# ZhongLingXiao/nano-kazen

Hardware: AMD Instinct MI355X
Metric: Msamples/s (w*h*spp/s) at 1920x1080, 1 M-tri scene (higher is better)
Workload: dtype f32

## Files before the change

### nano-kazen_amd/csrc/kz_render.hip

```cpp
#include <hip/hip_runtime.h>

#include "kz_devfn.h"
#include "kz_wavefront.h"
#include "kz_integrators.h"
#include "kz_aov.h"
#include "kz_state.h"
#include "../../include/kazen_mi355x_variance.h"
#include <algorithm>
#include <cmath>
#include <cstring>
#include <mutex>
#include <string>

template <bool STATS, int EXT>
__global__ __launch_bounds__(KZ_BLOCK) void kz_path_megakernel(KzParams P, KzDevTables T, const uint32_t *__restrict__ pixList,
                                                               uint32_t nItems, uint32_t S, uint32_t sampleBegin, const uint32_t *__restrict__ itemSample,
                                                               float *__restrict__ outJx, float *__restrict__ outJy, float *__restrict__ outR,
                                                               float *__restrict__ outG, float *__restrict__ outB,
                                                               unsigned long long *__restrict__ stats) {
    __shared__ uint32_t s_stack[KZ_STACK_DEPTH * KZ_BLOCK];
    const uint32_t item = blockIdx.x * KZ_BLOCK + threadIdx.x;
    Counters cn = {0, 0, 0, 0, 0, 0};
    if (item < nItems) {
        const uint32_t pl = item / S, so = item - pl * S;
// ... 24 lines not shown
}

static int stageMark(PassCtx &c, hipStream_t stream, int kind) {
    if (c.stageUsed == c.stageEv.size()) { Event e; if (const int rc = e.ensure()) return rc; c.stageEv.push_back(std::move(e)); c.stageKind.push_back(0); }
    c.stageKind[c.stageUsed] = kind;
    HIP_TRY(hipEventRecord(c.stageEv[c.stageUsed++], stream));
    return KZ_OK;
}

static constexpr size_t KZ_STATE_BYTES_PER_ITEM = 8 * sizeof(float4) + sizeof(uint4) + 3 * sizeof(uint32_t);
static constexpr size_t KZ_SAMPLE_BYTES_PER_ITEM = 5 * sizeof(float);

static void ctxPoint(PassCtx &c, const KzArena &A, size_t off) {
    KzWf W{};
    W.rayA.p = A.array<float4>(0) + off; W.rayB.p = A.array<float4>(1) + off; W.hit.p = A.array<float4>(2) + off; W.thr.p = A.array<float4>(3) + off;
    W.misc.p = A.array<float4>(4) + off; W.shA.p = A.array<float4>(5) + off; W.shB.p = A.array<float4>(6) + off; W.shL.p = A.array<float4>(7) + off;
    W.smp = A.array<uint4>(8) + off;
    for (int q = 0; q < 3; ++q) W.queue[q] = A.array<uint32_t>(9 + q) + off;
    W.counts = c.counts;
    c.wf = W;
    for (int k = 0; k < 5; ++k) c.plane[k] = A.array<float>(12 + k) + off;
}

static int ctxEnsure(PassCtx &c, size_t want, size_t minItems, double graceMs, hipStream_t stream, size_t *usable) {
    if (!c.counts) { if (const int rc = c.counts.alloc(KzCounts::kWords)) return rc; }
    KzArena &A = *c.arena;
    if (A.wouldReallocate(want)) HIP_TRY(hipDeviceSynchronize());
#ifdef KZ_EXPERIMENTS
    if (g_failAlloc > 0) { A.failCountdown.store(g_failAlloc); g_failAlloc = 0; }
#endif
    size_t got = 0;
    const int rc = A.request(want, minItems, graceMs, &got);
#ifdef KZ_EXPERIMENTS
    { std::lock_guard<std::mutex> g(A.m); if (!A.busy) g_failAlloc = A.failCountdown.exchange(0); }
#endif
    if (rc) return rc;
    ctxPoint(c, A, 0);
    *usable = std::min(got, want);
    return KZ_OK;
}

static decltype(&kz_wf_trace<0, false>) traceFn(int mode, bool stats) {
    static const decltype(&kz_wf_trace<0, false>) tab[5][2] = {{kz_wf_trace<0, false>, kz_wf_trace<0, true>}, {kz_wf_trace<1, false>, kz_wf_trace<1, true>},
                                        {kz_wf_trace<2, false>, kz_wf_trace<2, true>}, {nullptr, nullptr}, {kz_wf_trace<4, false>, kz_wf_trace<4, true>}};
#ifdef KZ_EXPERIMENTS
    if (mode == 4 && !g_kzShadowOrder.load(std::memory_order_relaxed)) return stats ? kz_wf_trace<5, true> : kz_wf_trace<5, false>;
#endif
    return tab[mode][stats ? 1 : 0];
}
static decltype(&kz_wf_trace_list<false, false>) listFn(bool stats, bool fix) {
    static const decltype(&kz_wf_trace_list<false, false>) tab[2][2] = {{kz_wf_trace_list<false, false>, kz_wf_trace_list<false, true>}, {kz_wf_trace_list<true, false>, kz_wf_trace_list<true, true>}};
    return tab[stats ? 1 : 0][fix ? 1 : 0];
}
static decltype(&kz_wf_trace_packet<false, false>) packetFn(bool stats, bool fix) {
    static const decltype(&kz_wf_trace_packet<false, false>) tab[2][2] = {{kz_wf_trace_packet<false, false>, kz_wf_trace_packet<false, true>}, {kz_wf_trace_packet<true, false>, kz_wf_trace_packet<true, true>}};
    return tab[stats ? 1 : 0][fix ? 1 : 0];
}
static int extSel(int bsdfExt, int all) { return bsdfExt == 0 ? 0 : (bsdfExt == KZ_X_MODELS ? KZ_X_MODELS : all); }
static int extCol(int ext) { return ext == 0 ? 0 : (ext == KZ_X_MODELS ? 1 : 2); }
typedef decltype(&kz_wf_shade<false, 0>) KzShadeFn;
static KzShadeFn shadeFn(bool stats, int ext) {
    static const KzShadeFn tab[2][3] = {{kz_wf_shade<false, 0>, kz_wf_shade<false, KZ_X_MODELS>, kz_wf_shade<false, KZ_X_ALL>}, {kz_wf_shade<true, 0>, kz_wf_shade<true, KZ_X_MODELS>, kz_wf_shade<true, KZ_X_ALL>}};
    return tab[stats ? 1 : 0][extCol(ext)];
}
typedef decltype(&kz_wf_mats<0>) KzMatsFn;
static KzMatsFn matsFn(int ext) {
    static const KzMatsFn tab[3] = {kz_wf_mats<0>, kz_wf_mats<KZ_X_MODELS>, kz_wf_mats<KZ_X_MATS>};
    return tab[extCol(ext)];
}
typedef decltype(&kz_path_megakernel<false, 0>) KzMegaFn;
static KzMegaFn megaFn(bool stats, int ext) {
    static const KzMegaFn tab[2][2] = {{kz_path_megakernel<false, 0>, kz_path_megakernel<false, KZ_X_ALL>}, {kz_path_megakernel<true, 0>, kz_path_megakernel<true, KZ_X_ALL>}};
    return tab[stats ? 1 : 0][ext ? 1 : 0];
}
typedef decltype(&kz_integrator_megakernel<KZ_INTEGRATOR_NORMALS, 0>) KzIntegratorMegaFn;
static KzIntegratorMegaFn integratorMegaFn(int integrator, int ext) {
    static const KzIntegratorMegaFn tab[3][2] = {{kz_integrator_megakernel<KZ_INTEGRATOR_NORMALS, 0>, kz_integrator_megakernel<KZ_INTEGRATOR_NORMALS, KZ_X_MATS>},
                                                 {kz_integrator_megakernel<KZ_INTEGRATOR_AO, 0>, kz_integrator_megakernel<KZ_INTEGRATOR_AO, KZ_X_MATS>},
                                                 {kz_integrator_megakernel<KZ_INTEGRATOR_PATH_MATS, 0>, kz_integrator_megakernel<KZ_INTEGRATOR_PATH_MATS, KZ_X_MATS>}};
    return tab[integrator == KZ_INTEGRATOR_NORMALS ? 0 : (integrator == KZ_INTEGRATOR_AO ? 1 : 2)][ext ? 1 : 0];
}

static int ensureBeamBuffers(KzScene *scene, KzDeviceState *ds, hipStream_t stream) {
    const KzParams &P = scene->prm;
    const size_t framePix = (size_t)P.width * P.height;
    int rc;
    if ((rc = ds->evBeam.ensure(hipEventDisableTiming))) return rc;
    if (!ds->beamEntries || !ds->beamCount) {
        if (!ds->beamEntries && (rc = ds->beamEntries.alloc(framePix * KZ_BEAM_CAP))) return rc;
        if (!ds->beamCount && (rc = ds->beamCount.alloc(framePix))) return rc;
        HIP_TRY(hipMemsetAsync(ds->beamCount, 0xFF, framePix * sizeof(uint2), stream));
        ds->beamDone.clear(); ds->beamDoneGen = ds->tileGen;
    }
    return KZ_OK;
}
static int ensureBeams(KzScene *scene, KzDeviceState *ds, hipStream_t stream, uint32_t p0, uint32_t n) {
    const KzParams &P = scene->prm;
    { const int rc_ = ensureBeamBuffers(scene, ds, stream); if (rc_) return rc_; }
    if (ds->beamDoneGen != ds->tileGen) { ds->beamDone.clear(); ds->beamDoneGen = ds->tileGen; }
    for (const auto &r : ds->beamDone) if (r.first <= p0 && p0 + n <= r.first + r.second) return KZ_OK;
    const int LS = std::max(1, std::min(P.stackBound4, KZ_BEAM_STACK));
    const dim3 gBeam((n + KZ_BLOCK - 1) / KZ_BLOCK);
    const size_t beamLds = (size_t)2 * LS * KZ_BLOCK * sizeof(uint32_t);
    hipLaunchKernelGGL(kz_wf_beam, gBeam, dim3(KZ_BLOCK), beamLds, stream, P, ds->T, (const uint32_t *)(ds->pixList + p0), n, LS, ds->beamEntries, ds->beamCount);
    if (ds->statsOn) hipLaunchKernelGGL(kz_wf_beam_count, gBeam, dim3(KZ_BLOCK), 0, stream, (const uint2 *)ds->beamCount, (const uint32_t *)(ds->pixList + p0), P.width, n, ds->stats + 24);
    HIP_TRY(hipGetLastError());
// ... 9 lines not shown
static bool packetFits(const KzParams &P) { return P.stackBound4 <= 128; }
struct TraceShape {
    int ldsStack;
    size_t traceLds;
    uint32_t ovfStride;
    size_t ovfRows, ovfPart;
};
static TraceShape traceShape(const KzParams &P, unsigned gridBlocks, int ldsStackAsked) {
    TraceShape s;
    const int stackBound = std::max(P.stackBound4, 2);
    s.ldsStack = std::max(2, std::min(ldsStackAsked, stackBound));
    s.traceLds = (size_t)(s.ldsStack + 1) * KZ_BLOCK * sizeof(uint32_t);
    s.ovfStride = (uint32_t)((size_t)gridBlocks * KZ_BLOCK);
    s.ovfRows = (size_t)std::max(1, stackBound - s.ldsStack);
    s.ovfPart = (size_t)s.ovfStride * s.ovfRows;
    return s;
}
static void launchTrace(int mode, bool stats, dim3 grid, size_t traceLds, hipStream_t on, const KzParams &P, const KzDevTables &T, const KzWf &W, const uint32_t *q, const uint32_t *cptr,
                        uint32_t cimm, uint32_t *head, KzTune t, uint32_t *qb, uint32_t *cb) {
    if (t.batch <= 0) t.batch = 128;
    if (t.refill <= 0) t.refill = (mode == 2 || mode == 4) ? 32 : 40;
    hipLaunchKernelGGL(traceFn(mode, stats), grid, dim3(KZ_BLOCK), traceLds, on, P, T, W, q, cptr, cimm, head, t, qb, cb);
}
template <class Trace>
static void shadowLaunches(const KzParams &P, Trace &&trace, const uint32_t *q, const uint32_t *cptr, uint32_t cimm, uint32_t *head, uint32_t *litQ, uint32_t *litCount, uint32_t *litHead) {
    if (P.shadowFast) {
        trace(4, q, cptr, cimm, head, litQ, litCount);
        if (P.anyInvisibleLight) trace(2, (const uint32_t *)litQ, (const uint32_t *)litCount, 0u, litHead, (uint32_t *)nullptr, (uint32_t *)nullptr);
    } else trace(2, q, cptr, cimm, head, (uint32_t *)nullptr, (uint32_t *)nullptr);
}

static int ensureOverflow(KzScene *scene, KzDeviceState *ds, PassCtx &c, const KzTune &tune, hipStream_t stream) {
    const size_t needOvf = traceShape(scene->prm, travGridBlocks(ds, tune), tune.ldsStack).ovfPart * 3;
    if (needOvf <= c.ovf.cap()) return KZ_OK;
    HIP_TRY(hipStreamSynchronize(stream));
    return c.ovf.regrow(needOvf);
}

struct WfLaunch {
    KzDeviceState *ds; PassCtx &c; hipStream_t stream;
    KzParams P; KzDevTables Tsh; KzWf W; KzTune tune;
    const uint32_t *pixList; uint32_t items, Sp, sBegin; bool st;
    dim3 blk, gItems, gTrav, gShade, gPacket;
    size_t traceLds, ovfPart;
    int mark(int kind) { return stageMark(c, stream, kind); }
    void trace(int mode, const uint32_t *q, const uint32_t *cptr, uint32_t cimm, uint32_t *head, uint32_t *qb, uint32_t *cb, hipStream_t on = nullptr) const {
        KzTune t = tune;
        const bool side = on != nullptr;
        if (side) t.ovf = tune.ovf + 2 * ovfPart; else on = stream;
        launchTrace(mode, st, gTrav, traceLds, on, P, ds->T, W, q, cptr, cimm, head, t, qb, cb);
    }
};

static int wfCamera(WfLaunch &L, bool beams) {
    const KzParams &P = L.P; const KzWf &W = L.W; KzDeviceState *ds = L.ds; hipStream_t stream = L.stream;
    uint32_t *cam = W.counts + KzCounts::kCamera, *fixCount = cam + KzCounts::kPaths;
    const bool packet = L.tune.packet != 1 && packetFits(P), fix = P.anyInvisibleLight != 0;
    if (packet && beams) {
        uint32_t *fbQ = W.queue[0], *fbCount = W.counts + KzCounts::kFallback, *fbHead = fbCount + 1;
        hipLaunchKernelGGL(listFn(L.st, fix), L.gItems, L.blk, 0, stream, P, ds->T, W, L.pixList, L.items, L.Sp, (const uint2 *)ds->beamEntries, (const uint2 *)ds->beamCount,
                           fbQ, fbCount, W.queue[2], fixCount);
        hipLaunchKernelGGL(packetFn(L.st, fix), L.gPacket, L.blk, 0, stream, P, ds->T, W, (const uint32_t *)fbQ, (const uint32_t *)fbCount, 0u, fbHead, KZ_PACKET_BATCH, W.queue[2], fixCount);
    } else if (packet) {
        hipLaunchKernelGGL(packetFn(L.st, fix), L.gPacket, L.blk, 0, stream, P, ds->T, W, (const uint32_t *)nullptr, (const uint32_t *)nullptr, L.items, cam + KzCounts::kBounceHead, KZ_PACKET_BATCH, W.queue[2], fixCount);
    } else {
        L.trace(0, nullptr, nullptr, L.items, cam + KzCounts::kBounceHead, nullptr, nullptr);
        if (fix) hipLaunchKernelGGL(kz_wf_primary_fix, L.gShade, L.blk, 0, stream, P, ds->T, W, L.items, W.queue[2], fixCount);
    }
    if (fix) L.trace(1, W.queue[2], fixCount, 0u, cam + KzCounts::kShadowHead, nullptr, nullptr);
    return L.mark(5);
}

#define KZ_VARIANCE_DEFAULT_ONE_PASS 1
static int filmStages(KzScene *scene, KzDeviceState *ds, hipStream_t pst, const uint32_t *pixList, uint32_t nPix, uint32_t Sp, const float *const plane[5], hipEvent_t waitFilm, int lanes) {
    const int mode = scene->varianceMode;
    if (!mode) return kzFilmStage(scene, ds, ds->picture(), false, pst, pixList, nPix, Sp, plane, waitFilm, lanes);
    const bool onePass = (mode == KZ_VARIANCE_ONE_PASS || (mode == KZ_VARIANCE_ON && KZ_VARIANCE_DEFAULT_ONE_PASS)) && kzFilmMomentOnePassOk(scene->prm);
    if (!onePass) if (const int rc = kzFilmStage(scene, ds, ds->picture(), false, pst, pixList, nPix, Sp, plane, waitFilm, lanes)) return rc;
    return kzFilmStageMoment(scene, ds, ds->picture(), ds->moment(), onePass, pst, pixList, nPix, Sp, plane, waitFilm);
}
static int filmLanes(const KzTune &tune) { return tune.filmGather == 3 ? 1 : 0; }
typedef decltype(&kz_wf_aov<0>) KzAovFn;
static KzAovFn aovFn(int ext) {
    static const KzAovFn tab[3] = {kz_wf_aov<0>, kz_wf_aov<KZ_X_MODELS>, kz_wf_aov<KZ_X_ALL>};
    return tab[extCol(ext)];
}
static int wfAov(KzScene *scene, WfLaunch &L, hipEvent_t waitAov, hipEvent_t recordAov) {
    const KzWf &W = L.W; hipStream_t stream = L.stream;
    static_assert(sizeof(float4) >= 3 * sizeof(float), "a shadow array holds three float planes per item");
    const KzAovPlanes A = {{(float *)W.shA.p, (float *)W.shB.p, (float *)W.shL.p}, (size_t)L.items};
    const dim3 grid(std::min(L.gItems.x, (unsigned)(L.ds->numCU * 8)));
    hipLaunchKernelGGL(aovFn(extSel(L.P.bsdfExt, KZ_X_ALL)), grid, L.blk, 0, stream, L.ds->T, W, L.items, scene->aovMask, A);
    HIP_TRY(hipGetLastError());
    if (waitAov) HIP_TRY(hipStreamWaitEvent(stream, waitAov, 0));
    for (int f = 0; f < 3; ++f) {
        if (!(scene->aovMask & (1u << f))) continue;
        KzFilm &film = L.ds->aov(f);
        if (!film.sums) return kz_fail(KZ_ERR_STATE, "the tap sums of AOV %u are not there", 1u << f);
        const float *const plane[5] = {W.outJx, W.outJy, A.p[f], A.p[f] + A.stride, A.p[f] + 2 * A.stride};
        if (const int rc = kzFilmStage(scene, L.ds, film, true, stream, L.pixList, L.items / L.Sp, L.Sp, plane, nullptr, filmLanes(L.tune))) return rc;
    }
    if (recordAov) HIP_TRY(hipEventRecord(recordAov, stream));
    return L.mark(4);
}

static int wfMats(WfLaunch &L) {
    int rc;
    const KzParams &P = L.P; const KzWf &W = L.W; hipStream_t stream = L.stream;
    const KzMatsFn mats = matsFn(extSel(P.bsdfExt, KZ_X_MATS));
    const uint32_t *cur = nullptr, *curCount = nullptr;
    for (int iter = 0; iter < P.maxDepth; ++iter) {
        uint32_t *nextQ = W.queue[iter & 1], *nextCount = W.counts + KzCounts::quad(iter);
        hipLaunchKernelGGL(mats, L.gShade, L.blk, 0, stream, P, L.ds->T, W, L.pixList, L.Sp, L.sBegin, iter, cur, curCount, cur ? 0u : L.items, nextQ, nextCount);
        if ((rc = L.mark(2))) return rc;
// ... 21 lines not shown
        uint32_t *nextQ = W.queue[iter & 1], *nextCount = W.counts + KzCounts::quad(iter), *shQ = W.queue[2], *shCount = nextCount + KzCounts::kShadows;
        hipLaunchKernelGGL(shade, L.gShade, L.blk, 0, stream, P, L.Tsh, W, L.pixList, L.Sp, L.sBegin, iter, cur, curCount, L.items, nextQ, nextCount, shQ, shCount);
        const bool needExtend = iter < P.maxDepth - 1 || P.bgPresent;
        if ((rc = L.mark(2))) return rc;
        hipStream_t shOn = nullptr;
        if (beside && needExtend) { HIP_TRY(hipEventRecord(c.evFork, stream)); HIP_TRY(hipStreamWaitEvent(c.side, c.evFork, 0)); shOn = c.side; }
        if (P.nLights > 0) {
            uint32_t *litQ = W.queue[(iter & 1) ^ 1], *litCount = W.counts + KzCounts::lit(iter), *litHead = litCount + 1;
            shadowLaunches(P, [&](int mode, const uint32_t *q, const uint32_t *cptr, uint32_t cimm, uint32_t *head, uint32_t *qb, uint32_t *cb) { L.trace(mode, q, cptr, cimm, head, qb, cb, shOn); },
                           shQ, shCount, 0u, nextCount + KzCounts::kShadowHead, litQ, litCount, litHead);
        }
        if (shOn) HIP_TRY(hipEventRecord(c.evJoin, c.side));
        if ((rc = L.mark(3))) return rc;
        if (needExtend) {
            L.trace(0, nextQ, nextCount, 0u, nextCount + KzCounts::kBounceHead, nullptr, nullptr);
            if (shOn) HIP_TRY(hipStreamWaitEvent(stream, c.evJoin, 0));
            if ((rc = L.mark(1))) return rc;
        }
        cur = nextQ; curCount = nextCount;
    }
    if (P.bgPresent) hipLaunchKernelGGL(kz_wf_final, L.gShade, L.blk, 0, stream, P, L.ds->T, W, cur, curCount);
    return KZ_OK;
}

static int wfPass(KzScene *scene, KzDeviceState *ds, PassCtx &c, hipStream_t stream, const uint32_t *pixList, uint32_t sBegin, uint32_t Sp, uint32_t items, KzTune tune, bool beams, bool beside,
                  hipEvent_t waitAov = nullptr, hipEvent_t recordAov = nullptr) {
    int rc;
    WfLaunch L{ds, c, stream};
    const bool mis = scene->prm.integrator == KZ_INTEGRATOR_PATH_MIS;
    KzParams &P = L.P = scene->prm;
    if (!mis) { P.anyInvisibleLight = 0; P.nIlTris = 0; P.shadowFast = 1; }
    L.Tsh = ds->T;
    if (ds->statsOn) L.Tsh.nEmTris = KZ_EM_OFF;
#ifdef KZ_EXPERIMENTS
    { const int mode = g_kzRrAhead.load(std::memory_order_relaxed);
      if (mode == 0) L.Tsh.nEmTris = KZ_EM_OFF; else if (mode == 2) L.Tsh.nEmTris = ds->T.nEmTris; }
#endif
    KzWf &W = L.W = c.wf;
    W.outJx = c.plane[0]; W.outJy = c.plane[1]; W.outR = c.plane[2]; W.outG = c.plane[3]; W.outB = c.plane[4]; W.stats = ds->stats;
    L.pixList = pixList; L.items = items; L.Sp = Sp; L.sBegin = sBegin; L.st = ds->statsOn;
    const int shadeBlocks = tune.shadeBlocksPerCU > 0 ? tune.shadeBlocksPerCU : !mis ? 8 : (P.bsdfExt ? 6 : KZ_SHADE_WAVES);
    L.blk = dim3(KZ_BLOCK); L.gItems = dim3((items + KZ_BLOCK - 1) / KZ_BLOCK);
    L.gTrav = dim3(travGridBlocks(ds, tune)); L.gShade = dim3((unsigned)(ds->numCU * shadeBlocks));
    L.gPacket = dim3(packetGridBlocks(ds));
    const TraceShape shape = traceShape(P, L.gTrav.x, tune.ldsStack);
    tune.ldsStack = shape.ldsStack;
    L.traceLds = shape.traceLds;
    if ((rc = ensureOverflow(scene, ds, c, tune, stream))) return rc;
    tune.ovf = c.ovf; tune.ovfStride = shape.ovfStride;
    L.tune = tune; L.ovfPart = shape.ovfPart;
    c.stageUsed = 0;
    HIP_TRY(hipMemsetAsync(W.counts, 0, KzCounts::bytes(), stream));
    if ((rc = L.mark(-1))) return rc;
    hipLaunchKernelGGL(kz_wf_generate, L.gItems, L.blk, 0, stream, P, ds->T, W, pixList, items, Sp, sBegin);
    if ((rc = L.mark(0))) return rc;
    if (mis && P.maxDepth <= 0 && !scene->aovMask) return KZ_OK;
    if ((rc = wfCamera(L, beams))) return rc;
    if (scene->aovMask && (rc = wfAov(scene, L, waitAov, recordAov))) return rc;
    if (mis && P.maxDepth <= 0) return KZ_OK;
    if (P.integrator == KZ_INTEGRATOR_NORMALS) {
        hipLaunchKernelGGL(kz_wf_normals, L.gShade, L.blk, 0, stream, P, ds->T, W, items);
        rc = L.mark(2);
    } else if (P.integrator == KZ_INTEGRATOR_AO) {
        uint32_t *quad = W.counts + KzCounts::quad(0), *shQ = W.queue[2], *shCount = quad + KzCounts::kShadows;
        hipLaunchKernelGGL(kz_wf_ao, L.gShade, L.blk, 0, stream, P, ds->T, W, pixList, Sp, sBegin, items, shQ, shCount);
        if ((rc = L.mark(2))) return rc;
        L.trace(4, shQ, shCount, 0u, quad + KzCounts::kShadowHead, nullptr, nullptr);
        rc = L.mark(3);
    } else rc = mis ? wfMis(L, beside) : wfMats(L);
    if (rc) return rc;
    if (L.st) hipLaunchKernelGGL(kz_wf_count, L.gItems, L.blk, 0, stream, W, items);
    HIP_TRY(hipGetLastError());
    return KZ_OK;
}

static int planIn(KzDeviceState *ds, const KzRenderOpts *opts, int pipeline, uint32_t s0, uint32_t s1, KzPlanIn &in) {
    in.pipeline = pipeline; in.nPix = ds->nPix; in.s0 = s0; in.s1 = s1;
    in.passItems = opts->passItems; in.passesInFlight = opts->passesInFlight; in.sppPerPass = opts->tune.sppPerPass;
    in.perItem = (pipeline == 2 ? KZ_STATE_BYTES_PER_ITEM : 0) + KZ_SAMPLE_BYTES_PER_ITEM;
    in.limit = opts->maxStateBytes;
    if (!in.limit) {
        size_t freeB = 0, totalB = 0;
        const size_t held = ds->ctxBytes() + kzCtxPoolBytes(ds->device);
        if (hipMemGetInfo(&freeB, &totalB) == hipSuccess && totalB > 0) in.limit = std::min(totalB / 4 * 3, freeB + held - std::min(freeB + held, KzArena::kRuntimeReserve + ((size_t)256 << 20)));
        else in.limit = (size_t)32 << 30;
        if (in.limit == 0) return kz_fail(KZ_ERR_OOM, "the device has %.2f GB free and this replica holds no pass context: nothing is left for path state beyond the %.2f GB a context leaves to the HIP runtime's own allocations",
                                          freeB / 1e9, (KzArena::kRuntimeReserve + ((size_t)256 << 20)) / 1e9);
    }
    const KzTileDealer *dealer = opts->dealer;
    in.dealer = dealer != nullptr;
    if (dealer) { in.takers = dealer->takers; in.dealerBatchTiles = dealer->batchTiles; in.nTiles = (uint32_t)ds->curTiles.size(); in.tilePixOffset = ds->tilePixOffset.data(); }
    in.heldBefore = ds->ctx[0] ? std::max(ds->ctx[0]->wanted, ds->ctx[0]->items()) : kzCtxPoolMaxItems(ds->device);
    return KZ_OK;
}

static int makeRoom(KzDeviceState *ds, int nCtx, size_t need, size_t perItem, size_t limit) {
    const size_t perCtx = need * perItem;
    size_t keep = 0;
    for (int i = 0; i < nCtx; ++i) { PassCtx &c = ds->ctxAt(i); if (c.arena) c.arena->lowerTarget(need); keep += std::max(c.bytes(), perCtx); }
    for (int i = KZ_MAX_PASSES_IN_FLIGHT - 1; i >= nCtx; --i) {
        if (!ds->ctx[i] || !ds->ctx[i]->bytes()) continue;
        if (keep + ds->ctx[i]->bytes() > limit) { HIP_TRY(hipDeviceSynchronize()); ds->ctx[i]->release(); } else keep += ds->ctx[i]->bytes();
    }
    if (keep + kzCtxPoolBytes(ds->device) > limit) (void)kzCtxPoolTrim(ds->device, limit > keep ? limit - keep : 0);
    if (keep > limit)
        for (int i = 0; i < nCtx; ++i) if (ds->ctx[i] && ds->ctx[i]->bytes() > perCtx) {
            HIP_TRY(hipDeviceSynchronize());
// ... 433 lines not shown
```

### nano-kazen_amd/csrc/kz_wavefront.h

```cpp
#pragma once
#include "kz_state.h"
#include "kz_devfn.h"

#ifndef KZ_WF_QCAP
#define KZ_WF_QCAP 960
#endif
#define KZ_WF_ROUNDS (KZ_WF_QCAP / KZ_BLOCK)

struct WfAppender {
    uint32_t *s_buf; uint32_t *s_n; uint32_t *s_gb; uint32_t *gQueue; uint32_t *gCount;
    __device__ __forceinline__ void push(bool pred, uint32_t val) {
        const unsigned long long m = __ballot(pred);
        const int lane = threadIdx.x & 63;
        uint32_t base = 0;
        if (lane == 0 && m) base = atomicAdd(s_n, (uint32_t)__popcll(m));
        base = __shfl(base, 0, 64);
        if (pred) s_buf[base + __popcll(m & ((1ull << lane) - 1ull))] = val;
    }
    __device__ __forceinline__ void maybeFlush(bool force) {
        __syncthreads();
        const uint32_t n = *s_n;
        if (force ? (n > 0) : (n > KZ_WF_QCAP - KZ_BLOCK)) {
            if (threadIdx.x == 0) *s_gb = atomicAdd(gCount, n);
            __syncthreads();
            const uint32_t gb = *s_gb;
            for (uint32_t i = threadIdx.x; i < n; i += KZ_BLOCK) gQueue[gb + i] = s_buf[i];
            __syncthreads();
            if (threadIdx.x == 0) *s_n = 0;
        }
        __syncthreads();
    }
};

__device__ __forceinline__ uint32_t wfPmjDim(const KzParams &P, int iter) {
    return 4u + (uint32_t)iter * (4u + (P.nLights > 0 ? 3u : 0u)) + (iter > 3 ? (uint32_t)(iter - 3) : 0u);
}
__device__ __forceinline__ void wfSampleOf(const uint32_t *__restrict__ pixList, uint32_t S, uint32_t sampleBegin, uint32_t slot, int &px, int &py, uint32_t &sampleIndex) {
    sampleIndex = sampleBegin + slot % S;
    pixelOf(pixList[slot / S], px, py);
}
__device__ __forceinline__ void wfLoadSampler(const KzParams &P, const KzWf &W, uint32_t slot, int px, int py, uint32_t sampleIndex, Sampler &s, uint32_t dimPmj) {
    s.type = P.samplerType; s.px = px; s.py = py; s.idx = sampleIndex;
    if (P.samplerType == KZ_SAMPLER_PMJ02BN) {
        s.state = 0ull; s.inc = 0ull; s.dim = dimPmj; s.hp = hashPixelBlock(px, py);
        return;
    }
    const uint4 v = W.smp[slot];
    s.state = (uint64_t)v.x | ((uint64_t)v.y << 32);
    s.dim = (uint32_t)__builtin_amdgcn_readfirstlane((int)v.z);
    s.inc = (P.samplerType == KZ_SAMPLER_PMJ02BN) ? 0ull : ((hashPixelSeed(px, py, P.seed) << 1u) | 1u);
    s.hp = (P.samplerType != KZ_SAMPLER_INDEPENDENT) ? hashPixelBlock(px, py) : 0ull;
}
__device__ __forceinline__ void wfStoreSampler(const KzParams &P, const KzWf &W, uint32_t slot, const Sampler &s) {
    uint4 v;
    if (P.samplerType == KZ_SAMPLER_PMJ02BN) return;
    v.x = (uint32_t)s.state; v.y = (uint32_t)(s.state >> 32); v.z = s.dim; v.w = 0;
    W.smp[slot] = v;
}
__device__ __forceinline__ void wfAddRadiance(const KzWf &W, uint32_t slot, V3 c) {
    unsafeAtomicAdd(W.outR + slot, c.x); unsafeAtomicAdd(W.outG + slot, c.y); unsafeAtomicAdd(W.outB + slot, c.z);
}
__device__ __forceinline__ void wfStoreWalkThrough(const KzParams &P, const KzWf &W, uint32_t slot, const Its &its, V3 d) {
    const V3 no = walkThroughOrigin(P, its, d);
    kzStoreStream(&W.shA[slot], make_float4(no.x, no.y, no.z, KZ_INF));
    kzStoreStream(&W.shB[slot], make_float4(d.x, d.y, d.z, KZ_EPSILON));
}

__global__ __launch_bounds__(KZ_BLOCK) void kz_wf_generate(KzParams P, KzDevTables T, KzWf W, const uint32_t *__restrict__ pixList,
                                                           uint32_t nItems, uint32_t S, uint32_t sampleBegin) {
    const uint32_t item = blockIdx.x * KZ_BLOCK + threadIdx.x;
    if (item >= nItems) return;
    uint32_t pl, pxy;
    if ((S & 63u) == 0) { pl = (uint32_t)__builtin_amdgcn_readfirstlane((int)item) / S; pxy = (uint32_t)__builtin_amdgcn_readfirstlane((int)pixList[pl]); }
    else { pl = item / S; pxy = pixList[pl]; }
    const uint32_t so = item - pl * S;
    int px, py; pixelOf(pxy, px, py);
    Sampler smp; smp.type = P.samplerType;
    smp.generateSample(P, T, px, py, sampleBegin + so);
    float jx, jy; smp.nextPixel2D(P, T, jx, jy);
    const float sx = (float)px + jx, sy = (float)py + jy;
    float ax, ay; smp.next2D(P, T, ax, ay);
    V3 ro, rd; float mint, maxt;
    cameraRay(P, sx, sy, ax, ay, ro, rd, mint, maxt);
    kzStoreStream(&W.rayA[item], make_float4(ro.x, ro.y, ro.z, mint));
    kzStoreStream(&W.rayB[item], make_float4(rd.x, rd.y, rd.z, maxt));
    wfStoreSampler(P, W, item, smp);
    W.outJx[item] = jx; W.outJy[item] = jy; W.outR[item] = 0.f; W.outG[item] = 0.f; W.outB[item] = 0.f;
}


__global__ __launch_bounds__(KZ_BLOCK) void kz_wf_primary_fix(KzParams P, KzDevTables T, KzWf W, uint32_t nItems, uint32_t *__restrict__ outQueue,
                                                              uint32_t *__restrict__ outCount) {
    __shared__ uint32_t s_buf[KZ_WF_QCAP]; __shared__ uint32_t s_n, s_gb;
    if (threadIdx.x == 0) s_n = 0;
    __syncthreads();
    WfAppender ap = {s_buf, &s_n, &s_gb, outQueue, outCount};
    for (uint32_t base = blockIdx.x * KZ_BLOCK; base < nItems; base += gridDim.x * KZ_BLOCK) {
        const uint32_t slot = base + threadIdx.x;
        bool need = false;
        if (slot < nItems) {
            const float4 h = kzLoadStream(&W.hit[slot]);
            if (h.x < KZ_INF) {
                const RawHit rh = rawHitOf(h);
                if (isInvisibleLight(T, lightOfGid(T, rh.gid))) {
                    Its its; postIntersect<false>(T, rh, its);
                    const float4 b = kzLoadStream(&W.rayB[slot]);
                    wfStoreWalkThrough(P, W, slot, its, mk(b.x, b.y, b.z));
                    need = true;
                }
            }
        }
        ap.push(need, slot);
        ap.maybeFlush(false);
    }
    ap.maybeFlush(true);
}

#ifndef KZ_SHADE_WAVES
#define KZ_SHADE_WAVES 4
#endif
struct KzSst {
#ifdef KZ_SHADESTAT
    unsigned long long t = __builtin_amdgcn_s_memtime(), acc[14] = {0, 0, 0, 0, 0, 0, 0, 0, 0, 0, 0, 0, 0, 0};
    __device__ __forceinline__ void mark(int k) { const unsigned long long t_ = __builtin_amdgcn_s_memtime(); acc[k] += t_ - t; t = t_; }
    __device__ __forceinline__ void markw(int k) { __builtin_amdgcn_s_waitcnt(0); mark(k); }
    __device__ __forceinline__ void flush(unsigned long long *stats) { if ((threadIdx.x & 63) == 0) for (int k = 0; k < 14; ++k) atomicAdd(stats + 8 + k, acc[k]); }
#else
    __device__ __forceinline__ void mark(int) {}
    __device__ __forceinline__ void markw(int) {}
    __device__ __forceinline__ void flush(unsigned long long *) {}
#endif
};

__device__ __forceinline__ bool wfEmitterBox(const KzDevTables &T, V3 o, V3 d, float tmin) {
    const float rx = rcpExact(d.x), ry = rcpExact(d.y), rz = rcpExact(d.z);
    float t0 = (T.emLo[0] - o.x) * rx, t1 = (T.emHi[0] - o.x) * rx;
    float n = fminf(t0, t1), f = fmaxf(t0, t1);
    t0 = (T.emLo[1] - o.y) * ry; t1 = (T.emHi[1] - o.y) * ry; n = fmaxf(n, fminf(t0, t1)); f = fminf(f, fmaxf(t0, t1));
    t0 = (T.emLo[2] - o.z) * rz; t1 = (T.emHi[2] - o.z) * rz; n = fmaxf(n, fminf(t0, t1)); f = fminf(f, fmaxf(t0, t1));
    f *= 1.0000004f;
// ... 673 lines not shown
    auto popMin = [&]() -> bool {
        if (n == 0) return false;
        int im = 0; uint32_t km = kst[0];
        for (int i = 1; i < n; ++i) { const uint32_t k = kst[i * KZ_BLOCK]; if (k < km) { km = k; im = i; } }
        if (!(__uint_as_float(km) < tvalid)) return false;
        cur = stk[im * KZ_BLOCK]; curKey = __uint_as_float(km);
        --n;
        if (im != n) { stk[im * KZ_BLOCK] = stk[n * KZ_BLOCK]; kst[im * KZ_BLOCK] = kst[n * KZ_BLOCK]; }
        return true;
    };
    while (__any(active)) {
        bool needPop = false;
        if (active && !(cur & 0x80000000u)) {
            const uint4 *np = kzNode4Ptr(T, cur);
            const uint4 q0 = np[0], q1 = np[1], q2 = np[2], refs = np[3];
            const float sX = __uint_as_float(q0.w), sY = __uint_as_float(q2.z), sZ = __uint_as_float(q2.w);
            const float pX = __uint_as_float(q0.x) - O.x, pY = __uint_as_float(q0.y) - O.y, pZ = __uint_as_float(q0.z) - O.z;
            const uint32_t r[4] = {refs.x, refs.y, refs.z, refs.w};
#pragma unroll
            for (int i = 0; i < 4; ++i) {
                const float qlx = (float)((q1.x >> (8 * i)) & 0xffu), qly = (float)((q1.y >> (8 * i)) & 0xffu), qlz = (float)((q1.z >> (8 * i)) & 0xffu);
                const float qhx = (float)((q1.w >> (8 * i)) & 0xffu), qhy = (float)((q2.x >> (8 * i)) & 0xffu), qhz = (float)((q2.y >> (8 * i)) & 0xffu);
                const float lx = fmaf(qlx, sX, pX), ly = fmaf(qly, sY, pY), lz = fmaf(qlz, sZ, pZ), hx = fmaf(qhx, sX, pX), hy = fmaf(qhy, sY, pY), hz = fmaf(qhz, sZ, pZ);
                const float reach = fmaxf(fabsf(lx), fabsf(hx)) + fmaxf(fabsf(ly), fabsf(hy)) + fmaxf(fabsf(lz), fabsf(hz));
                const float pad = rho * reach + 1.9e-6f * (reach + fabsf(O.x) + fabsf(O.y) + fabsf(O.z));
                const float t0x = (lx - pad) * rx, t1x = (hx + pad) * rx, t0y = (ly - pad) * ry, t1y = (hy + pad) * ry, t0z = (lz - pad) * rz, t1z = (hz + pad) * rz;
                const float nn = fmaxf(fmaxf(fminf(t0x, t1x), fminf(t0y, t1y)), fmaxf(fminf(t0z, t1z), 0.f));
                const float ff = fminf(fminf(fmaxf(t0x, t1x), fmaxf(t0y, t1y)), fmaxf(t0z, t1z)) * 1.0000004f;
                const float key = fmaxf(nn * 0.999999f, curKey);
                if (qhx >= qlx && nn <= ff && key < tvalid) push(r[i], __float_as_uint(key));
            }
            needPop = true;
        } else if (active) {
            if (count < KZ_BEAM_CAP) { myList[count] = make_uint2(cur, __float_as_uint(curKey)); ++count; needPop = true; }
            else { tvalid = fminf(tvalid, curKey); active = false; }
        }
        if (needPop && !popMin()) active = false;
    }
    if (todo) heads[fpix] = make_uint2(count, __float_as_uint(tvalid));
}

__global__ __launch_bounds__(KZ_BLOCK) void kz_wf_beam_count(const uint2 *__restrict__ heads, const uint32_t *__restrict__ pixList, int width, uint32_t nPix, unsigned long long *__restrict__ out) {
    const uint32_t pl = blockIdx.x * KZ_BLOCK + threadIdx.x;
    uint2 h = make_uint2(0u, 0u);
    if (pl < nPix) h = heads[framePixelOf(pixList[pl], (uint32_t)width)];
    unsigned long long v[3] = {pl < nPix ? 1ull : 0ull, (unsigned long long)h.x, (pl < nPix && !(__uint_as_float(h.y) < KZ_INF)) ? 1ull : 0ull};
    for (int k = 0; k < 3; ++k) {
        unsigned long long x = v[k];
        for (int off = 32; off > 0; off >>= 1) x += __shfl_down(x, off, 64);
        if ((threadIdx.x & 63) == 0 && x) atomicAdd(&out[k], x);
    }
}

template <bool STATS, bool FIX>
__global__ __launch_bounds__(KZ_BLOCK) void kz_wf_trace_list(KzParams P, KzDevTables T, KzWf W, const uint32_t *__restrict__ pixList, uint32_t nItems, uint32_t S, const uint2 *__restrict__ entries,
                                                             const uint2 *__restrict__ heads, uint32_t *__restrict__ fbQueue, uint32_t *__restrict__ fbCount,
                                                             uint32_t *__restrict__ fixQueue, uint32_t *__restrict__ fixCount) {
    const uint32_t slot = blockIdx.x * KZ_BLOCK + threadIdx.x;
    const int lane = threadIdx.x & 63;
    Counters cn = {0, 0, 0, 0, 0, 0};
    const bool have = slot < nItems;
    bool undecided = false;
    if (have) {
        const uint32_t pl = (S & 63u) == 0 ? (uint32_t)__builtin_amdgcn_readfirstlane((int)slot) / S : slot / S;
        const float4 a = kzLoadStream(&W.rayA[slot]), b = kzLoadStream(&W.rayB[slot]);
        const V3 o = mk(a.x, a.y, a.z), d = mk(b.x, b.y, b.z);
        const float tmin = a.w;
        float tmax = b.w;
        bool found = false; float bt = KZ_INF, bu = 0.f, bv = 0.f; uint32_t bgid = 0;
        const bool finite = rayIsFinite(o, d);
        const float len = sqrtf(dot(d, d)), lenUp = len * 1.000002f;
        float tvalidDist = KZ_INF;
        auto consider = [&](float t, float u, float v, uint32_t g) { if (!found || t < bt || (t == bt && g < bgid)) { found = true; bt = t; bu = u; bv = v; bgid = g; tmax = t; } };
        auto walk = [&](const uint2 *__restrict__ lst, const uint2 head) {
            tvalidDist = __uint_as_float(head.y);
            if (!finite) return;
            for (uint32_t j = 0; j < head.x; ++j) {
                const uint2 e = lst[j];
                if (__uint_as_float(e.y) > tmax * lenUp) continue;
                const uint32_t start = (e.x & 0x7fffffffu) >> 3, cnt = (e.x & 7u) + 1;
                for (uint32_t i = 0; i < cnt; ++i) {
                    float t, u, v; uint32_t g;
                    if (STATS) cn.tris++;
                    if (triTest(T.tris + start + i, o, d, tmin, tmax, t, u, v, g)) consider(t, u, v, g);
                }
            }
        };
        auto walkShared = [&](const uint2 *__restrict__ lst, const uint2 head) {
            tvalidDist = __uint_as_float(head.y);
            if (!finite || head.x == 0) return;
            uint2 e = lst[0];
            for (uint32_t j = 0; j < head.x; ++j) {
                const uint2 eNext = lst[min(j + 1u, head.x - 1u)];
                const bool inFront = __uint_as_float(e.y) <= tmax * lenUp;
                if (!__any(inFront)) break;
                if (inFront) {
                    const uint32_t start = (e.x & 0x7fffffffu) >> 3, cnt = (e.x & 7u) + 1;
                    for (uint32_t i = 0; i < cnt; i += 2) {
                        const float4 *tp = reinterpret_cast<const float4 *>(T.tris + start + i), *tq = tp + (i + 1 < cnt ? 3 : 0);
                        const float4 a0 = tp[0], b0 = tp[1], c0 = tp[2], a1 = tq[0], b1 = tq[1], c1 = tq[2];
                        float t, u, v; uint32_t g;
                        if (STATS) cn.tris++;
                        if (triTestV(a0, b0, c0, o, d, tmin, tmax, t, u, v, g)) consider(t, u, v, g);
                        if (i + 1 < cnt) {
                            if (STATS) cn.tris++;
                            if (triTestV(a1, b1, c1, o, d, tmin, tmax, t, u, v, g)) consider(t, u, v, g);
                        }
                    }
                }
                e = eNext;
            }
        };
        const uint32_t plU = (uint32_t)__builtin_amdgcn_readfirstlane((int)pl);
        if (__all(pl == plU)) { const uint32_t fp = framePixelOf(pixList[plU], (uint32_t)P.width); walkShared(entries + (size_t)fp * KZ_BEAM_CAP, heads[fp]); }
        else { const uint32_t fp = framePixelOf(pixList[pl], (uint32_t)P.width); walk(entries + (size_t)fp * KZ_BEAM_CAP, heads[fp]); }
        undecided = finite && !(found ? bt * lenUp < tvalidDist : !(tvalidDist < KZ_INF));
        if (STATS && !undecided) cn.rays++;
        if (undecided) {
            kzStoreStream(&W.rayA[slot], make_float4(a.x, a.y, a.z, fmaxf(tmin, tvalidDist / lenUp * 0.999998f)));
            if (found) kzStoreStream(&W.rayB[slot], make_float4(b.x, b.y, b.z, bt));
        } else {
            kzStoreStream(&W.hit[slot], make_float4(bt, bu, bv, __uint_as_float(bgid)))        ;
            if (FIX && found && bgid - P.ilGidLo <= P.ilGidSpan) {
                if (isInvisibleLight(T, lightOfGid(T, bgid))) {
                    const RawHit rh = rawHitOf(bt, bu, bv, bgid);
                    Its its; postIntersect<false>(T, rh, its);
                    wfStoreWalkThrough(P, W, slot, its, d);
                    fixQueue[atomicAdd(fixCount, 1u)] = slot;
                }
            }
        }
    }
    {
        const unsigned long long m = __ballot(undecided);
        if (m) {
            uint32_t base = 0;
            if (lane == 0) base = atomicAdd(fbCount, (uint32_t)__popcll(m));
            base = (uint32_t)__builtin_amdgcn_readfirstlane((int)base);
            if (undecided) fbQueue[base + __builtin_amdgcn_mbcnt_hi((uint32_t)(m >> 32), __builtin_amdgcn_mbcnt_lo((uint32_t)m, 0u))] = slot;
        }
    }
    if (STATS) statsFlush(W.stats, cn, 0);
}

__global__ __launch_bounds__(KZ_BLOCK) void kz_wf_final(KzParams P, KzDevTables T, KzWf W, const uint32_t *__restrict__ queue, const uint32_t *__restrict__ countPtr) {
    const uint32_t count = *countPtr;
    for (uint32_t qi = blockIdx.x * KZ_BLOCK + threadIdx.x; qi < count; qi += gridDim.x * KZ_BLOCK) {
        const uint32_t slot = queue[qi];
        const float4 h = kzLoadStream(&W.hit[slot]);
        if (h.x < KZ_INF) continue;
        const float4 rb = kzLoadStream(&W.rayB[slot]), th = kzLoadStream(&W.thr[slot]);
        const V3 bg = backgroundRadiance(P, T, mk(rb.x, rb.y, rb.z));
        unsafeAtomicAdd(W.outR + slot, th.x * bg.x); unsafeAtomicAdd(W.outG + slot, th.y * bg.y); unsafeAtomicAdd(W.outB + slot, th.z * bg.z);
    }
}

__global__ __launch_bounds__(KZ_BLOCK) void kz_wf_count(KzWf W, uint32_t nItems) {
    Counters cn = {0, 0, 0, 0, 0, 0};
    const uint32_t i = blockIdx.x * KZ_BLOCK + threadIdx.x;
    if (i < nItems) {
        const float r = W.outR[i], g = W.outG[i], b = W.outB[i];
        if (!(r >= 0 && g >= 0 && b >= 0 && isfinite(r) && isfinite(g) && isfinite(b))) cn.dropped++;
    }
    statsFlush(W.stats, cn, i < nItems ? 1u : 0u);
}
```

Measured before the change: 1940.

## Fuse camera ray generation into beam-list primary trace kernel

Adds a kz_wf_camera kernel that generates the camera ray and immediately walks the per-pixel beam list, keeping the ray in registers instead of writing rayA/rayB and reading them back in a separate kernel. It is enabled by default when packet tracing with beams is used, and the separate generate launch is skipped in that case. This removes one kernel launch and one global round trip of ray data per sample. In exchange the fused kernel always writes the ray (even when decided), and the fused kernel's register pressure is constrained by the waves_per_eu attribute.

```diff
diff --git a/nano-kazen_amd/csrc/kz_render.hip b/nano-kazen_amd/csrc/kz_render.hip
--- a/nano-kazen_amd/csrc/kz_render.hip
+++ b/nano-kazen_amd/csrc/kz_render.hip
@@ -100,6 +100,10 @@
     static const decltype(&kz_wf_trace_list<false, false>) tab[2][2] = {{kz_wf_trace_list<false, false>, kz_wf_trace_list<false, true>}, {kz_wf_trace_list<true, false>, kz_wf_trace_list<true, true>}};
     return tab[stats ? 1 : 0][fix ? 1 : 0];
 }
+static decltype(&kz_wf_camera<false, false>) cameraFn(bool stats, bool fix) {
+    static const decltype(&kz_wf_camera<false, false>) tab[2][2] = {{kz_wf_camera<false, false>, kz_wf_camera<false, true>}, {kz_wf_camera<true, false>, kz_wf_camera<true, true>}};
+    return tab[stats ? 1 : 0][fix ? 1 : 0];
+}
 static decltype(&kz_wf_trace_packet<false, false>) packetFn(bool stats, bool fix) {
     static const decltype(&kz_wf_trace_packet<false, false>) tab[2][2] = {{kz_wf_trace_packet<false, false>, kz_wf_trace_packet<false, true>}, {kz_wf_trace_packet<true, false>, kz_wf_trace_packet<true, true>}};
     return tab[stats ? 1 : 0][fix ? 1 : 0];
@@ -215,14 +219,25 @@
     }
 };
 
+#ifndef KZ_CAMERA_FUSED_DEFAULT
+#define KZ_CAMERA_FUSED_DEFAULT 1
+#endif
+static bool cameraPacket(const KzTune &tune, const KzParams &P) { return tune.packet != 1 && packetFits(P); }
+static bool cameraFused(const KzTune &tune, const KzParams &P, bool beams) {
+    return beams && cameraPacket(tune, P) && (tune.packet == 4 || (tune.packet != 3 && KZ_CAMERA_FUSED_DEFAULT));
+}
 static int wfCamera(WfLaunch &L, bool beams) {
     const KzParams &P = L.P; const KzWf &W = L.W; KzDeviceState *ds = L.ds; hipStream_t stream = L.stream;
     uint32_t *cam = W.counts + KzCounts::kCamera, *fixCount = cam + KzCounts::kPaths;
-    const bool packet = L.tune.packet != 1 && packetFits(P), fix = P.anyInvisibleLight != 0;
+    const bool packet = cameraPacket(L.tune, P), fix = P.anyInvisibleLight != 0;
     if (packet && beams) {
         uint32_t *fbQ = W.queue[0], *fbCount = W.counts + KzCounts::kFallback, *fbHead = fbCount + 1;
-        hipLaunchKernelGGL(listFn(L.st, fix), L.gItems, L.blk, 0, stream, P, ds->T, W, L.pixList, L.items, L.Sp, (const uint2 *)ds->beamEntries, (const uint2 *)ds->beamCount,
-                           fbQ, fbCount, W.queue[2], fixCount);
+        if (cameraFused(L.tune, P, beams))
+            hipLaunchKernelGGL(cameraFn(L.st, fix), L.gItems, L.blk, 0, stream, P, ds->T, W, L.pixList, L.items, L.Sp, L.sBegin, (const uint2 *)ds->beamEntries, (const uint2 *)ds->beamCount,
+                               fbQ, fbCount, W.queue[2], fixCount);
+        else
+            hipLaunchKernelGGL(listFn(L.st, fix), L.gItems, L.blk, 0, stream, P, ds->T, W, L.pixList, L.items, L.Sp, (const uint2 *)ds->beamEntries, (const uint2 *)ds->beamCount,
+                               fbQ, fbCount, W.queue[2], fixCount);
         hipLaunchKernelGGL(packetFn(L.st, fix), L.gPacket, L.blk, 0, stream, P, ds->T, W, (const uint32_t *)fbQ, (const uint32_t *)fbCount, 0u, fbHead, KZ_PACKET_BATCH, W.queue[2], fixCount);
     } else if (packet) {
         hipLaunchKernelGGL(packetFn(L.st, fix), L.gPacket, L.blk, 0, stream, P, ds->T, W, (const uint32_t *)nullptr, (const uint32_t *)nullptr, L.items, cam + KzCounts::kBounceHead, KZ_PACKET_BATCH, W.queue[2], fixCount);
@@ -350,7 +365,7 @@
     c.stageUsed = 0;
     HIP_TRY(hipMemsetAsync(W.counts, 0, KzCounts::bytes(), stream));
     if ((rc = L.mark(-1))) return rc;
-    hipLaunchKernelGGL(kz_wf_generate, L.gItems, L.blk, 0, stream, P, ds->T, W, pixList, items, Sp, sBegin);
+    if (!cameraFused(tune, P, beams)) hipLaunchKernelGGL(kz_wf_generate, L.gItems, L.blk, 0, stream, P, ds->T, W, pixList, items, Sp, sBegin);
     if ((rc = L.mark(0))) return rc;
     if (mis && P.maxDepth <= 0 && !scene->aovMask) return KZ_OK;
     if ((rc = wfCamera(L, beams))) return rc;
diff --git a/nano-kazen_amd/csrc/kz_wavefront.h b/nano-kazen_amd/csrc/kz_wavefront.h
--- a/nano-kazen_amd/csrc/kz_wavefront.h
+++ b/nano-kazen_amd/csrc/kz_wavefront.h
@@ -66,11 +66,10 @@
     kzStoreStream(&W.shB[slot], make_float4(d.x, d.y, d.z, KZ_EPSILON));
 }
 
-__global__ __launch_bounds__(KZ_BLOCK) void kz_wf_generate(KzParams P, KzDevTables T, KzWf W, const uint32_t *__restrict__ pixList,
-                                                           uint32_t nItems, uint32_t S, uint32_t sampleBegin) {
-    const uint32_t item = blockIdx.x * KZ_BLOCK + threadIdx.x;
-    if (item >= nItems) return;
-    uint32_t pl, pxy;
+template <bool STORE_RAY>
+__device__ __forceinline__ void wfGenerateItem(const KzParams &P, const KzDevTables &T, const KzWf &W, const uint32_t *__restrict__ pixList, uint32_t item, uint32_t S,
+                                               uint32_t sampleBegin, uint32_t &pl, V3 &ro, V3 &rd, float &mint, float &maxt) {
+    uint32_t pxy;
     if ((S & 63u) == 0) { pl = (uint32_t)__builtin_amdgcn_readfirstlane((int)item) / S; pxy = (uint32_t)__builtin_amdgcn_readfirstlane((int)pixList[pl]); }
     else { pl = item / S; pxy = pixList[pl]; }
     const uint32_t so = item - pl * S;
@@ -80,12 +79,20 @@
     float jx, jy; smp.nextPixel2D(P, T, jx, jy);
     const float sx = (float)px + jx, sy = (float)py + jy;
     float ax, ay; smp.next2D(P, T, ax, ay);
-    V3 ro, rd; float mint, maxt;
     cameraRay(P, sx, sy, ax, ay, ro, rd, mint, maxt);
-    kzStoreStream(&W.rayA[item], make_float4(ro.x, ro.y, ro.z, mint));
-    kzStoreStream(&W.rayB[item], make_float4(rd.x, rd.y, rd.z, maxt));
+    if (STORE_RAY) {
+        kzStoreStream(&W.rayA[item], make_float4(ro.x, ro.y, ro.z, mint));
+        kzStoreStream(&W.rayB[item], make_float4(rd.x, rd.y, rd.z, maxt));
+    }
     wfStoreSampler(P, W, item, smp);
     W.outJx[item] = jx; W.outJy[item] = jy; W.outR[item] = 0.f; W.outG[item] = 0.f; W.outB[item] = 0.f;
+}
+__global__ __launch_bounds__(KZ_BLOCK) void kz_wf_generate(KzParams P, KzDevTables T, KzWf W, const uint32_t *__restrict__ pixList,
+                                                           uint32_t nItems, uint32_t S, uint32_t sampleBegin) {
+    const uint32_t item = blockIdx.x * KZ_BLOCK + threadIdx.x;
+    if (item >= nItems) return;
+    uint32_t pl; V3 ro, rd; float mint, maxt;
+    wfGenerateItem<true>(P, T, W, pixList, item, S, sampleBegin, pl, ro, rd, mint, maxt);
 }
 
 
@@ -865,94 +872,120 @@
     }
 }
 
+template <bool STATS, bool FIX, bool IN_REGS>
+__device__ __forceinline__ bool wfListItem(const KzParams &P, const KzDevTables &T, const KzWf &W, const uint32_t *__restrict__ pixList, uint32_t slot, uint32_t pl, const float4 a, const float4 b,
+                                           const uint2 *__restrict__ entries, const uint2 *__restrict__ heads, uint32_t *__restrict__ fixQueue, uint32_t *__restrict__ fixCount, Counters &cn) {
+    const V3 o = mk(a.x, a.y, a.z), d = mk(b.x, b.y, b.z);
+    const float tmin = a.w;
+    float tmax = b.w;
+    bool found = false; float bt = KZ_INF, bu = 0.f, bv = 0.f; uint32_t bgid = 0;
+    const bool finite = rayIsFinite(o, d);
+    const float len = sqrtf(dot(d, d)), lenUp = len * 1.000002f;
+    float tvalidDist = KZ_INF;
+    auto consider = [&](float t, float u, float v, uint32_t g) { if (!found || t < bt || (t == bt && g < bgid)) { found = true; bt = t; bu = u; bv = v; bgid = g; tmax = t; } };
+    auto walk = [&](const uint2 *__restrict__ lst, const uint2 head) {
+        tvalidDist = __uint_as_float(head.y);
+        if (!finite) return;
+        for (uint32_t j = 0; j < head.x; ++j) {
+            const uint2 e = lst[j];
+            if (__uint_as_float(e.y) > tmax * lenUp) continue;
+            const uint32_t start = (e.x & 0x7fffffffu) >> 3, cnt = (e.x & 7u) + 1;
+            for (uint32_t i = 0; i < cnt; ++i) {
+                float t, u, v; uint32_t g;
+                if (STATS) cn.tris++;
+                if (triTest(T.tris + start + i, o, d, tmin, tmax, t, u, v, g)) consider(t, u, v, g);
+            }
+        }
+    };
+    auto walkShared = [&](const uint2 *__restrict__ lst, const uint2 head) {
+        tvalidDist = __uint_as_float(head.y);
+        if (!finite || head.x == 0) return;
+        uint2 e = lst[0];
+        for (uint32_t j = 0; j < head.x; ++j) {
+            const uint2 eNext = lst[min(j + 1u, head.x - 1u)];
+            const bool inFront = __uint_as_float(e.y) <= tmax * lenUp;
+            if (!__any(inFront)) break;
+            if (inFront) {
+                const uint32_t start = (e.x & 0x7fffffffu) >> 3, cnt = (e.x & 7u) + 1;
+                for (uint32_t i = 0; i < cnt; i += 2) {
+                    const float4 *tp = reinterpret_cast<const float4 *>(T.tris + start + i), *tq = tp + (i + 1 < cnt ? 3 : 0);
+                    const float4 a0 = tp[0], b0 = tp[1], c0 = tp[2], a1 = tq[0], b1 = tq[1], c1 = tq[2];
+                    float t, u, v; uint32_t g;
+                    if (STATS) cn.tris++;
+                    if (triTestV(a0, b0, c0, o, d, tmin, tmax, t, u, v, g)) consider(t, u, v, g);
+                    if (i + 1 < cnt) {
+                        if (STATS) cn.tris++;
+                        if (triTestV(a1, b1, c1, o, d, tmin, tmax, t, u, v, g)) consider(t, u, v, g);
+                    }
+                }
+            }
+            e = eNext;
+        }
+    };
+    const uint32_t plU = (uint32_t)__builtin_amdgcn_readfirstlane((int)pl);
+    if (__all(pl == plU)) { const uint32_t fp = framePixelOf(pixList[plU], (uint32_t)P.width); walkShared(entries + (size_t)fp * KZ_BEAM_CAP, heads[fp]); }
+    else { const uint32_t fp = framePixelOf(pixList[pl], (uint32_t)P.width); walk(entries + (size_t)fp * KZ_BEAM_CAP, heads[fp]); }
+    const bool undecided = finite && !(found ? bt * lenUp < tvalidDist : !(tvalidDist < KZ_INF));
+    if (STATS && !undecided) cn.rays++;
+    if (IN_REGS) {
+        kzStoreStream(&W.rayA[slot], make_float4(a.x, a.y, a.z, undecided ? fmaxf(tmin, tvalidDist / lenUp * 0.999998f) : a.w));
+        kzStoreStream(&W.rayB[slot], make_float4(b.x, b.y, b.z, undecided && found ? bt : b.w));
+    } else if (undecided) {
+        kzStoreStream(&W.rayA[slot], make_float4(a.x, a.y, a.z, fmaxf(tmin, tvalidDist / lenUp * 0.999998f)));
+        if (found) kzStoreStream(&W.rayB[slot], make_float4(b.x, b.y, b.z, bt));
+    }
+    if (!undecided) {
+        kzStoreStream(&W.hit[slot], make_float4(bt, bu, bv, __uint_as_float(bgid)))        ;
+        if (FIX && found && bgid - P.ilGidLo <= P.ilGidSpan) {
+            if (isInvisibleLight(T, lightOfGid(T, bgid))) {
+                const RawHit rh = rawHitOf(bt, bu, bv, bgid);
+                Its its; postIntersect<false>(T, rh, its);
+                wfStoreWalkThrough(P, W, slot, its, d);
+                fixQueue[atomicAdd(fixCount, 1u)] = slot;
+            }
+        }
+    }
+    return undecided;
+}
+__device__ __forceinline__ void wfAppendUndecided(bool undecided, uint32_t slot, uint32_t *__restrict__ fbQueue, uint32_t *__restrict__ fbCount) {
+    const int lane = threadIdx.x & 63;
+    const unsigned long long m = __ballot(undecided);
+    if (m) {
+        uint32_t base = 0;
+        if (lane == 0) base = atomicAdd(fbCount, (uint32_t)__popcll(m));
+        base = (uint32_t)__builtin_amdgcn_readfirstlane((int)base);
+        if (undecided) fbQueue[base + __builtin_amdgcn_mbcnt_hi((uint32_t)(m >> 32), __builtin_amdgcn_mbcnt_lo((uint32_t)m, 0u))] = slot;
+    }
+}
 template <bool STATS, bool FIX>
 __global__ __launch_bounds__(KZ_BLOCK) void kz_wf_trace_list(KzParams P, KzDevTables T, KzWf W, const uint32_t *__restrict__ pixList, uint32_t nItems, uint32_t S, const uint2 *__restrict__ entries,
                                                              const uint2 *__restrict__ heads, uint32_t *__restrict__ fbQueue, uint32_t *__restrict__ fbCount,
                                                              uint32_t *__restrict__ fixQueue, uint32_t *__restrict__ fixCount) {
     const uint32_t slot = blockIdx.x * KZ_BLOCK + threadIdx.x;
-    const int lane = threadIdx.x & 63;
     Counters cn = {0, 0, 0, 0, 0, 0};
-    const bool have = slot < nItems;
     bool undecided = false;
-    if (have) {
+    if (slot < nItems) {
         const uint32_t pl = (S & 63u) == 0 ? (uint32_t)__builtin_amdgcn_readfirstlane((int)slot) / S : slot / S;
         const float4 a = kzLoadStream(&W.rayA[slot]), b = kzLoadStream(&W.rayB[slot]);
-        const V3 o = mk(a.x, a.y, a.z), d = mk(b.x, b.y, b.z);
-        const float tmin = a.w;
-        float tmax = b.w;
-        bool found = false; float bt = KZ_INF, bu = 0.f, bv = 0.f; uint32_t bgid = 0;
-        const bool finite = rayIsFinite(o, d);
-        const float len = sqrtf(dot(d, d)), lenUp = len * 1.000002f;
-        float tvalidDist = KZ_INF;
-        auto consider = [&](float t, float u, float v, uint32_t g) { if (!found || t < bt || (t == bt && g < bgid)) { found = true; bt = t; bu = u; bv = v; bgid = g; tmax = t; } };
-        auto walk = [&](const uint2 *__restrict__ lst, const uint2 head) {
-            tvalidDist = __uint_as_float(head.y);
-            if (!finite) return;
-            for (uint32_t j = 0; j < head.x; ++j) {
-                const uint2 e = lst[j];
-                if (__uint_as_float(e.y) > tmax * lenUp) continue;
-                const uint32_t start = (e.x & 0x7fffffffu) >> 3, cnt = (e.x & 7u) + 1;
-                for (uint32_t i = 0; i < cnt; ++i) {
-                    float t, u, v; uint32_t g;
-                    if (STATS) cn.tris++;
-                    if (triTest(T.tris + start + i, o, d, tmin, tmax, t, u, v, g)) consider(t, u, v, g);
-                }
-            }
-        };
-        auto walkShared = [&](const uint2 *__restrict__ lst, const uint2 head) {
-            tvalidDist = __uint_as_float(head.y);
-            if (!finite || head.x == 0) return;
-            uint2 e = lst[0];
-            for (uint32_t j = 0; j < head.x; ++j) {
-                const uint2 eNext = lst[min(j + 1u, head.x - 1u)];
-                const bool inFront = __uint_as_float(e.y) <= tmax * lenUp;
-                if (!__any(inFront)) break;
-                if (inFront) {
-                    const uint32_t start = (e.x & 0x7fffffffu) >> 3, cnt = (e.x & 7u) + 1;
-                    for (uint32_t i = 0; i < cnt; i += 2) {
-                        const float4 *tp = reinterpret_cast<const float4 *>(T.tris + start + i), *tq = tp + (i + 1 < cnt ? 3 : 0);
-                        const float4 a0 = tp[0], b0 = tp[1], c0 = tp[2], a1 = tq[0], b1 = tq[1], c1 = tq[2];
-                        float t, u, v; uint32_t g;
-                        if (STATS) cn.tris++;
-                        if (triTestV(a0, b0, c0, o, d, tmin, tmax, t, u, v, g)) consider(t, u, v, g);
-                        if (i + 1 < cnt) {
-                            if (STATS) cn.tris++;
-                            if (triTestV(a1, b1, c1, o, d, tmin, tmax, t, u, v, g)) consider(t, u, v, g);
-                        }
-                    }
-                }
-                e = eNext;
-            }
-        };
-        const uint32_t plU = (uint32_t)__builtin_amdgcn_readfirstlane((int)pl);
-        if (__all(pl == plU)) { const uint32_t fp = framePixelOf(pixList[plU], (uint32_t)P.width); walkShared(entries + (size_t)fp * KZ_BEAM_CAP, heads[fp]); }
-        else { const uint32_t fp = framePixelOf(pixList[pl], (uint32_t)P.width); walk(entries + (size_t)fp * KZ_BEAM_CAP, heads[fp]); }
-        undecided = finite && !(found ? bt * lenUp < tvalidDist : !(tvalidDist < KZ_INF));
-        if (STATS && !undecided) cn.rays++;
-        if (undecided) {
-            kzStoreStream(&W.rayA[slot], make_float4(a.x, a.y, a.z, fmaxf(tmin, tvalidDist / lenUp * 0.999998f)));
-            if (found) kzStoreStream(&W.rayB[slot], make_float4(b.x, b.y, b.z, bt));
-        } else {
-            kzStoreStream(&W.hit[slot], make_float4(bt, bu, bv, __uint_as_float(bgid)))        ;
-            if (FIX && found && bgid - P.ilGidLo <= P.ilGidSpan) {
-                if (isInvisibleLight(T, lightOfGid(T, bgid))) {
-                    const RawHit rh = rawHitOf(bt, bu, bv, bgid);
-                    Its its; postIntersect<false>(T, rh, its);
-                    wfStoreWalkThrough(P, W, slot, its, d);
-                    fixQueue[atomicAdd(fixCount, 1u)] = slot;
-                }
-            }
-        }
-    }
-    {
-        const unsigned long long m = __ballot(undecided);
-        if (m) {
-            uint32_t base = 0;
-            if (lane == 0) base = atomicAdd(fbCount, (uint32_t)__popcll(m));
-            base = (uint32_t)__builtin_amdgcn_readfirstlane((int)base);
-            if (undecided) fbQueue[base + __builtin_amdgcn_mbcnt_hi((uint32_t)(m >> 32), __builtin_amdgcn_mbcnt_lo((uint32_t)m, 0u))] = slot;
-        }
-    }
+        undecided = wfListItem<STATS, FIX, false>(P, T, W, pixList, slot, pl, a, b, entries, heads, fixQueue, fixCount, cn);
+    }
+    wfAppendUndecided(undecided, slot, fbQueue, fbCount);
+    if (STATS) statsFlush(W.stats, cn, 0);
+}
+
+template <bool STATS, bool FIX>
+__global__ __launch_bounds__(KZ_BLOCK) __attribute__((amdgpu_waves_per_eu(8, 8))) void kz_wf_camera(KzParams P, KzDevTables T, KzWf W, const uint32_t *__restrict__ pixList, uint32_t nItems, uint32_t S,
+                                                         uint32_t sampleBegin, const uint2 *__restrict__ entries, const uint2 *__restrict__ heads, uint32_t *__restrict__ fbQueue,
+                                                         uint32_t *__restrict__ fbCount, uint32_t *__restrict__ fixQueue, uint32_t *__restrict__ fixCount) {
+    const uint32_t item = blockIdx.x * KZ_BLOCK + threadIdx.x;
+    Counters cn = {0, 0, 0, 0, 0, 0};
+    bool undecided = false;
+    if (item < nItems) {
+        uint32_t pl; V3 ro, rd; float mint, maxt;
+        wfGenerateItem<false>(P, T, W, pixList, item, S, sampleBegin, pl, ro, rd, mint, maxt);
+        undecided = wfListItem<STATS, FIX, true>(P, T, W, pixList, item, pl, make_float4(ro.x, ro.y, ro.z, mint), make_float4(rd.x, rd.y, rd.z, maxt), entries, heads, fixQueue, fixCount, cn);
+    }
+    wfAppendUndecided(undecided, item, fbQueue, fbCount);
     if (STATS) statsFlush(W.stats, cn, 0);
 }
 
```

New measurement: 1953 (median of 6 runs). No clear change (+0.7%).
